# Edresson/VoiceSplit

Measured on AMD Instinct MI355X. Metric: utterances/sec (3 s clips, B=64/GPU) fwd+bwd, channels-last bf16 activations / tape, bf16 MFMA, fp32 accumulate / statistics / master weights, higher is better.
Workload: dtype bf16 (conv activations and tape stored as bf16; bf16 MFMA operands in the convs, the LSTM / head contractions and the BPTT, f16 operands in the forward recurrence; fp32 accumulate, BatchNorm statistics, gate arithmetic / cell state, loss head, master weights)

## Files before the change

### voicesplit_amd/csrc/lstm.hip

```cpp
#include "vs_internal.h"

namespace {

typedef unsigned u32x4_t __attribute__((ext_vector_type(4)));

__global__ void lstm_pack_whh_kernel(const float* __restrict__ whh_f, const float* __restrict__ whh_b,
                                     float* __restrict__ wp, int H) {
  const int HQ = H / 8;
  const long long total = 2LL * HQ * HQ * 256;
  long long idx = (long long)blockIdx.x * blockDim.x + threadIdx.x;
  if (idx >= total) return;
  const int j = idx & 3;
  const int lane = (idx >> 2) & 63;
  long long rest = idx >> 8;
  const int q = rest % HQ; rest /= HQ;
  const int jg = rest % HQ;
  const int dir = rest / HQ;
  const int i = lane & 31;
  const int row = (i >> 3) * H + jg * 8 + (i & 7);
  const int k = 8 * q + 2 * j + (lane >> 5);
  const float* w = dir ? whh_b : whh_f;
  wp[idx] = w[(size_t)row * H + k];
}

// ... 721 lines not shown
    if (s > 0) {
      if (wave == 0 && !sDead) {
        unsigned spins = 0;
        for (;;) {
          bool ok = true;
          for (int j = lane; j < HQ; j += 64)
            ok = ok && (__hip_atomic_load(gflags + j, __ATOMIC_RELAXED, __HIP_MEMORY_SCOPE_AGENT) >= (unsigned)s);
          if (__all(ok)) break;
          if (++spins > kSpinLimit) {
            if (lane == 0) { sDead = 1; __hip_atomic_store(a.err, 1u, __ATOMIC_RELAXED, __HIP_MEMORY_SCOPE_AGENT); }
            break;
          }
          __builtin_amdgcn_s_sleep(1);
        }
      }
      __syncthreads();
      const unsigned hoff = (unsigned)((group * NC * NP * 64 + lane) * 16);
      f16x8 h[kMaxC][NP];
#pragma unroll
      for (int i = 0; i < kMaxC; ++i) {
        const int c = wave + 4 * i;
#pragma unroll
        for (int p = 0; p < NP; ++p)
          h[i][p] = __builtin_bit_cast(f16x8, c < NC ? __builtin_amdgcn_raw_buffer_load_b128(hrs[s & 1], hoff + (unsigned)(c * NP + p) * 1024u, 0, 16 )
                                                       : u32x4_t{0u, 0u, 0u, 0u});
      }
#pragma unroll
      for (int i = 0; i < kMaxC; ++i) {
        if (wave + 4 * i < NC) {
          if (NP == 2) {
            acc = __builtin_amdgcn_mfma_f32_32x32x16_f16(w[i][NP - 1], h[i][0], acc, 0, 0, 0);
            acc = __builtin_amdgcn_mfma_f32_32x32x16_f16(w[i][0], h[i][NP - 1], acc, 0, 0, 0);
          }
          acc = __builtin_amdgcn_mfma_f32_32x32x16_f16(w[i][0], h[i][0], acc, 0, 0, 0);
        }
      }
      for (int c = wave + 4 * kMaxC; c < NC; c += 4) {
        f16x8 wc[NP], hc[NP];
#pragma unroll
        for (int p = 0; p < NP; ++p) {
          wc[p] = __builtin_bit_cast(f16x8, wq[(size_t)(c * NP + p) * 64]);
          hc[p] = __builtin_bit_cast(f16x8, __builtin_amdgcn_raw_buffer_load_b128(hrs[s & 1], hoff + (unsigned)(c * NP + p) * 1024u, 0, 16));
        }
        if (NP == 2) {
          acc = __builtin_amdgcn_mfma_f32_32x32x16_f16(wc[NP - 1], hc[0], acc, 0, 0, 0);
          acc = __builtin_amdgcn_mfma_f32_32x32x16_f16(wc[0], hc[NP - 1], acc, 0, 0, 0);
        }
        acc = __builtin_amdgcn_mfma_f32_32x32x16_f16(wc[0], hc[0], acc, 0, 0, 0);
      }
    }
    if (wave > 0) {
#pragma unroll
      for (int r = 0; r < 16; ++r) sRed[((wave - 1) * 16 + r) * 64 + lane] = acc[r];
    }
    __syncthreads();
    if (wave == 0) {
#pragma unroll
      for (int w3 = 0; w3 < 3; ++w3)
#pragma unroll
        for (int r = 0; r < 16; ++r) acc[r] += sRed[(w3 * 16 + r) * 64 + lane];
      float hv[4], cnew[4], gact[4][4];
#pragma unroll
      for (int u = 0; u < 4; ++u) {
        const float gi = vs_sigmoid_fast(fmaf(acc[0 + u], inv, xgv[0 + u]));
        const float gf = vs_sigmoid_fast(fmaf(acc[4 + u], inv, xgv[4 + u]));
        const float gg = vs_tanh_fast(fmaf(acc[8 + u], inv, xgv[8 + u]));
        const float go = vs_sigmoid_fast(fmaf(acc[12 + u], inv, xgv[12 + u]));
        const float cn = gf * cprev[u] + gi * gg;
        hv[u] = go * vs_tanh_fast(cn);
        cnew[u] = cn;
        cprev[u] = cn;
        gact[0][u] = gi; gact[1][u] = gf; gact[2][u] = gg; gact[3][u] = go;
      }
      {
        float full[8];
#pragma unroll
        for (int u = 0; u < 4; ++u) {
          const float o = __shfl_xor(hv[u], 32, 64);
          full[u] = half ? o : hv[u];
          full[4 + u] = half ? hv[u] : o;
        }
        u32x4_t v;
        typedef _Float16 h2 __attribute__((ext_vector_type(2)));
#pragma unroll
        for (int j = 0; j < 4; ++j) {
          if (NP == 2) {
            const float x0 = full[2 * j] * kHScale, x1 = full[2 * j + 1] * kHScale;
            const h2 hh = __builtin_bit_cast(h2, __builtin_amdgcn_cvt_pkrtz(x0, x1));
            const unsigned lo = __builtin_bit_cast(unsigned, __builtin_amdgcn_cvt_pkrtz(x0 - (float)hh[0], x1 - (float)hh[1]));
            v[j] = half ? lo : __builtin_bit_cast(unsigned, hh);
          } else {
            const h2 hh = {(_Float16)full[2 * j], (_Float16)full[2 * j + 1]};
            v[j] = __builtin_bit_cast(unsigned, hh);
          }
        }
        const unsigned plane = NP == 2 ? (unsigned)half : 0u;
        const unsigned off = (unsigned)((((group * NC + (jg >> 1)) * NP + plane) * 64 + (jg & 1) * 32 + l31) * 16);
        if (NP == 2 || half == 0)
          __builtin_amdgcn_raw_buffer_store_b128(v, hrs[(s + 1) & 1], off, 0, 16 );
      }
      asm volatile("s_waitcnt vmcnt(0)" ::: "memory");
      if (lane == 0) __hip_atomic_store(gflags + jg, (unsigned)(s + 1), __ATOMIC_RELAXED, __HIP_MEMORY_SCOPE_AGENT);
      if (b < a.B) {
        float4* o = reinterpret_cast<float4*>(a.out + ((size_t)b * a.T + t) * (2 * a.H) + (size_t)dir * a.H + jg * 8 + 4 * half);
        *o = make_float4(hv[0], hv[1], hv[2], hv[3]);
        if (a.c_save) {
          float4* cs = reinterpret_cast<float4*>(a.c_save + ((size_t)b * a.T + t) * (2 * a.H) + (size_t)dir * a.H + jg * 8 + 4 * half);
          *cs = make_float4(cnew[0], cnew[1], cnew[2], cnew[3]);
        }
        if (a.gates_save) {
          float* grow = a.gates_save + ((size_t)b * a.T + t) * (8 * a.H) + (size_t)dir * 4 * a.H + jg * 8 + 4 * half;
#pragma unroll
          for (int gq = 0; gq < 4; ++gq)
            *reinterpret_cast<float4*>(grow + gq * a.H) = make_float4(gact[gq][0], gact[gq][1], gact[gq][2], gact[gq][3]);
        }
      }
    }
  }
}

constexpr unsigned kSentinel = 0x7FFF7FFFu;

template <int NP, bool RAGGED>
__global__ __launch_bounds__(256)
void lstm16_tagged_kernel(Lstm16Args a, void* hbuf2, void* hbuf3, const int* __restrict__ lengths) {
  __shared__ float sRed[2][3 * 16 * 64];
  __shared__ int sDead;
  const int tid = threadIdx.x;
  const int lane = tid & 63;
  const int wave = __builtin_amdgcn_readfirstlane(tid >> 6);
  const int l31 = lane & 31, half = lane >> 5;
  const int HQ = a.H / 8;
  const int NC = (a.H + 15) / 16;
  const int NBT = a.Bpad / 32;
  const int jg = blockIdx.x % HQ;
  const int bt = a.bt0 + blockIdx.x / HQ;
  const int dir = blockIdx.y;
  const int b = bt * 32 + l31;
  if (tid == 0) sDead = 0;

  const u32x4_t* wq = a.wp + ((size_t)(dir * HQ + jg) * NC * NP) * 64 + lane;
  f16x8 w[kMaxC][NP];
  bool owned[kMaxC];
#pragma unroll
  for (int i = 0; i < kMaxC; ++i) {
    const int c = wave + 4 * i;
    owned[i] = c < NC && 16 * c + 8 * half < a.H;
#pragma unroll
    for (int p = 0; p < NP; ++p)
      w[i][p] = __builtin_bit_cast(f16x8, c < NC ? wq[(size_t)(c * NP + p) * 64] : u32x4_t{0u, 0u, 0u, 0u});
  }
  const float inv = a.hdr[0];
  const size_t group = (size_t)dir * NBT + bt;
  const unsigned hbytes = (unsigned)((size_t)2 * NBT * NC * NP * 1024);
  __amdgpu_buffer_rsrc_t hrs[4] = {__builtin_amdgcn_make_buffer_rsrc(a.hbuf0, 0, hbytes, 0x00020000),
                                   __builtin_amdgcn_make_buffer_rsrc(a.hbuf1, 0, hbytes, 0x00020000),
                                   __builtin_amdgcn_make_buffer_rsrc(hbuf2, 0, hbytes, 0x00020000),
                                   __builtin_amdgcn_make_buffer_rsrc(hbuf3, 0, hbytes, 0x00020000)};
  const unsigned plane = NP == 2 ? (unsigned)half : 0u;
  const unsigned slot_off = (unsigned)((((group * NC + (jg >> 1)) * NP + plane) * 64 + (jg & 1) * 32 + l31) * 16);
  const bool storer = NP == 2 || half == 0;
  float cprev[4] = {0.f, 0.f, 0.f, 0.f};
  int len = a.T;
  if (RAGGED) len = b < a.B ? lengths[b] : 0;
  __syncthreads();

#pragma unroll 1
  for (int s = 0; s < a.T; ++s) {
    const int t = dir ? (a.T - 1 - s) : s;
    const int rb = s & 3, wb = (s + 1) & 3, zb = (s + 3) & 3;
    float xgv[16];
    if (wave == 0) {
      const bool ok = b < a.B;
      const float* xrow = a.xg + ((size_t)(ok ? b : 0) * a.T + t) * (8 * a.H) + (size_t)dir * 4 * a.H + jg * 8 + 4 * half;
#pragma unroll
      for (int r = 0; r < 16; ++r) xgv[r] = ok ? xrow[(r >> 2) * a.H + (r & 3)] : 0.f;
    }
    f32x16 acc;
#pragma unroll
    for (int r = 0; r < 16; ++r) acc[r] = 0.f;
    if (s > 0) {
      const unsigned hoff = (unsigned)((group * NC * NP * 64 + lane) * 16);
      f16x8 h[kMaxC][NP];
      unsigned spins = 0;
      for (;;) {
        bool ok = true;
#pragma unroll
        for (int i = 0; i < kMaxC; ++i) {
          const int c = wave + 4 * i;
#pragma unroll
          for (int p = 0; p < NP; ++p) {
            u32x4_t v = c < NC ? __builtin_amdgcn_raw_buffer_load_b128(hrs[rb], hoff + (unsigned)(c * NP + p) * 1024u, 0, 16 )
                               : u32x4_t{0u, 0u, 0u, 0u};
            if (!owned[i]) v = u32x4_t{0u, 0u, 0u, 0u};
            ok = ok && v[0] != kSentinel && v[1] != kSentinel && v[2] != kSentinel && v[3] != kSentinel;
            h[i][p] = __builtin_bit_cast(f16x8, v);
          }
        }
        if (__all(ok)) break;
        if (++spins > kSpinLimit / 4 || *(volatile int*)&sDead) {
          if (lane == 0) { sDead = 1; __hip_atomic_store(a.err, 1u, __ATOMIC_RELAXED, __HIP_MEMORY_SCOPE_AGENT); }
          break;
        }
        __builtin_amdgcn_s_sleep(1);
      }
#pragma unroll
      for (int i = 0; i < kMaxC; ++i) {
        if (wave + 4 * i < NC) {
          if (NP == 2) {
            acc = __builtin_amdgcn_mfma_f32_32x32x16_f16(w[i][NP - 1], h[i][0], acc, 0, 0, 0);
            acc = __builtin_amdgcn_mfma_f32_32x32x16_f16(w[i][0], h[i][NP - 1], acc, 0, 0, 0);
          }
          acc = __builtin_amdgcn_mfma_f32_32x32x16_f16(w[i][0], h[i][0], acc, 0, 0, 0);
        }
      }
    }
    if (wave > 0) {
#pragma unroll
      for (int r = 0; r < 16; ++r) sRed[s & 1][((wave - 1) * 16 + r) * 64 + lane] = acc[r];
    }
    if (wave == 1) asm volatile("s_waitcnt vmcnt(0)" ::: "memory");
    __syncthreads();
    if (wave == 1 && s > 0 && storer)
      __builtin_amdgcn_raw_buffer_store_b128(u32x4_t{kSentinel, kSentinel, kSentinel, kSentinel}, hrs[zb], slot_off, 0, 16);
    if (wave == 0) {
#pragma unroll
      for (int w3 = 0; w3 < 3; ++w3)
#pragma unroll
        for (int r = 0; r < 16; ++r) acc[r] += sRed[s & 1][(w3 * 16 + r) * 64 + lane];
      float hv[4], cnew[4], gact[4][4];
#pragma unroll
      for (int u = 0; u < 4; ++u) {
        const float gi = vs_sigmoid_fast(fmaf(acc[0 + u], inv, xgv[0 + u]));
        const float gf = vs_sigmoid_fast(fmaf(acc[4 + u], inv, xgv[4 + u]));
        const float gg = vs_tanh_fast(fmaf(acc[8 + u], inv, xgv[8 + u]));
        const float go = vs_sigmoid_fast(fmaf(acc[12 + u], inv, xgv[12 + u]));
        float cn = gf * cprev[u] + gi * gg;
        hv[u] = go * vs_tanh_fast(cn);
        if (RAGGED) {
          cn = t < len ? cn : 0.f;
          hv[u] = t < len ? hv[u] : 0.f;
        }
        cnew[u] = cn;
        cprev[u] = cn;
        gact[0][u] = gi; gact[1][u] = gf; gact[2][u] = gg; gact[3][u] = go;
      }
      {
        float full[8];
#pragma unroll
        for (int u = 0; u < 4; ++u) {
          const float o = __shfl_xor(hv[u], 32, 64);
          full[u] = half ? o : hv[u];
          full[4 + u] = half ? hv[u] : o;
        }
        u32x4_t v;
        typedef _Float16 h2 __attribute__((ext_vector_type(2)));
#pragma unroll
        for (int j = 0; j < 4; ++j) {
          if (NP == 2) {
            const float x0 = full[2 * j] * kHScale, x1 = full[2 * j + 1] * kHScale;
            const h2 hh = __builtin_bit_cast(h2, __builtin_amdgcn_cvt_pkrtz(x0, x1));
            const unsigned lo = __builtin_bit_cast(unsigned, __builtin_amdgcn_cvt_pkrtz(x0 - (float)hh[0], x1 - (float)hh[1]));
            v[j] = half ? lo : __builtin_bit_cast(unsigned, hh);
          } else {
            const h2 hh = {(_Float16)full[2 * j], (_Float16)full[2 * j + 1]};
            v[j] = __builtin_bit_cast(unsigned, hh);
          }
          v[j] = v[j] == kSentinel ? 0x7FFF7E00u : v[j];
        }
        if (storer) __builtin_amdgcn_raw_buffer_store_b128(v, hrs[wb], slot_off, 0, 16 );
      }
      if (b < a.B) {
        float4* o = reinterpret_cast<float4*>(a.out + ((size_t)b * a.T + t) * (2 * a.H) + (size_t)dir * a.H + jg * 8 + 4 * half);
        *o = make_float4(hv[0], hv[1], hv[2], hv[3]);
        if (a.c_save) {
          float4* cs = reinterpret_cast<float4*>(a.c_save + ((size_t)b * a.T + t) * (2 * a.H) + (size_t)dir * a.H + jg * 8 + 4 * half);
          *cs = make_float4(cnew[0], cnew[1], cnew[2], cnew[3]);
        }
        if (a.gates_save) {
          float* grow = a.gates_save + ((size_t)b * a.T + t) * (8 * a.H) + (size_t)dir * 4 * a.H + jg * 8 + 4 * half;
#pragma unroll
          for (int gq = 0; gq < 4; ++gq)
            *reinterpret_cast<float4*>(grow + gq * a.H) = make_float4(gact[gq][0], gact[gq][1], gact[gq][2], gact[gq][3]);
        }
      }
    }
  }
}

struct Lstm16BwdArgs {
  const u32x4_t* wpt;
  void* gbuf0;
  void* gbuf1;
  unsigned* flags;
  unsigned* err;
  float* gates;
  const float* c_all;
  const float* dout;
  int B, T, H, Bpad, bt0;
};

constexpr int kBwdRes16 = 13;

__global__ __launch_bounds__(512)
void lstm16_bwd_persistent_kernel(Lstm16BwdArgs a) {
  __shared__ float sRed[8 * 16 * 64];
  __shared__ int sDead;
  const int tid = threadIdx.x;
  const int lane = tid & 63;
  const int wave = __builtin_amdgcn_readfirstlane(tid >> 6);
  const int half = lane >> 5;
  const int NCt = a.H / 4;
  const int NUT = (a.H + 31) / 32;
  const int NBT = a.Bpad / 32;
  const int ut = blockIdx.x % NUT;
  const int bt = a.bt0 + blockIdx.x / NUT;
  const int dir = blockIdx.y;
  if (tid == 0) sDead = 0;

  const int b31 = tid & 31, ug = (tid >> 5) & 7;
  const int b = bt * 32 + b31;
  const int u0 = ut * 32 + 4 * ug;
  const bool units_ok = tid < 256 && u0 < a.H;
  const bool item = units_ok && b < a.B;

  const u32x4_t* wq = a.wpt + ((size_t)(dir * NUT + ut) * NCt) * 64 + lane;
  bf16x8 w[kBwdRes16];
#pragma unroll
  for (int i = 0; i < kBwdRes16; ++i) {
    const int c = wave + 8 * i;
    w[i] = __builtin_bit_cast(bf16x8, c < NCt ? wq[(size_t)c * 64] : u32x4_t{0u, 0u, 0u, 0u});
  }
  const size_t group = (size_t)dir * NBT + bt;
  const unsigned gbytes = (unsigned)((size_t)2 * NBT * NCt * 1024);
  __amdgpu_buffer_rsrc_t grs[2] = {__builtin_amdgcn_make_buffer_rsrc(a.gbuf0, 0, gbytes, 0x00020000),
                                   __builtin_amdgcn_make_buffer_rsrc(a.gbuf1, 0, gbytes, 0x00020000)};
  const int nflag = NUT * 4;
  unsigned* const gflags = a.flags + group * nflag;
  float dcc[4] = {0.f, 0.f, 0.f, 0.f};
  __syncthreads();

#pragma unroll 1
  for (int s = 0; s < a.T; ++s) {
    const int t = dir ? s : (a.T - 1 - s);
    const int tp = dir ? t + 1 : t - 1;
    float4 gi4, gf4, gg4, go4, c4, cp4, dh4;
    gi4 = gf4 = gg4 = go4 = c4 = cp4 = dh4 = make_float4(0.f, 0.f, 0.f, 0.f);
    float* grow = a.gates + ((size_t)(item ? b : 0) * a.T + t) * (8 * a.H) + (size_t)dir * 4 * a.H + (item ? u0 : 0);
    if (item) {
      gi4 = *reinterpret_cast<const float4*>(grow);
      gf4 = *reinterpret_cast<const float4*>(grow + a.H);
      gg4 = *reinterpret_cast<const float4*>(grow + 2 * a.H);
      go4 = *reinterpret_cast<const float4*>(grow + 3 * a.H);
      const size_t so = ((size_t)b * a.T + t) * (2 * a.H) + (size_t)dir * a.H + u0;
      c4 = *reinterpret_cast<const float4*>(a.c_all + so);
      dh4 = *reinterpret_cast<const float4*>(a.dout + so);
      if (tp >= 0 && tp < a.T)
        cp4 = *reinterpret_cast<const float4*>(a.c_all + ((size_t)b * a.T + tp) * (2 * a.H) + (size_t)dir * a.H + u0);
    }
    f32x16 acc;
#pragma unroll
    for (int r = 0; r < 16; ++r) acc[r] = 0.f;
    if (s > 0) {
      if (wave == 0 && !sDead) {
        unsigned spins = 0;
        for (;;) {
          bool ok = true;
          for (int j = lane; j < nflag; j += 64)
            ok = ok && (__hip_atomic_load(gflags + j, __ATOMIC_RELAXED, __HIP_MEMORY_SCOPE_AGENT) >= (unsigned)s);
          if (__all(ok)) break;
          if (++spins > kSpinLimit) {
            if (lane == 0) { sDead = 1; __hip_atomic_store(a.err, 1u, __ATOMIC_RELAXED, __HIP_MEMORY_SCOPE_AGENT); }
            break;
          }
          __builtin_amdgcn_s_sleep(1);
        }
      }
      __syncthreads();
      const unsigned goff = (unsigned)((group * NCt * 64 + lane) * 16);
      bf16x8 g[kBwdRes16];
#pragma unroll
      for (int i = 0; i < kBwdRes16; ++i) {
        const int c = wave + 8 * i;
        g[i] = __builtin_bit_cast(bf16x8, c < NCt ? __builtin_amdgcn_raw_buffer_load_b128(grs[s & 1], goff + (unsigned)c * 1024u, 0, 16 )
                                                  : u32x4_t{0u, 0u, 0u, 0u});
      }
#pragma unroll
      for (int i = 0; i < kBwdRes16; ++i) {
        if (wave + 8 * i < NCt)
          acc = __builtin_amdgcn_mfma_f32_32x32x16_bf16(w[i], g[i], acc, 0, 0, 0);
      }
      for (int c = wave + 8 * kBwdRes16; c < NCt; c += 8) {
        const bf16x8 wc = __builtin_bit_cast(bf16x8, wq[(size_t)c * 64]);
        const bf16x8 gc = __builtin_bit_cast(bf16x8, __builtin_amdgcn_raw_buffer_load_b128(grs[s & 1], goff + (unsigned)c * 1024u, 0, 16));
        acc = __builtin_amdgcn_mfma_f32_32x32x16_bf16(wc, gc, acc, 0, 0, 0);
      }
    }
#pragma unroll
    for (int r = 0; r < 16; ++r) sRed[(wave * 16 + r) * 64 + lane] = acc[r];
    __syncthreads();
    if (tid < 256) {
      float dh[4] = {dh4.x, dh4.y, dh4.z, dh4.w};
#pragma unroll
      for (int w8 = 0; w8 < 8; ++w8)
#pragma unroll
        for (int u = 0; u < 4; ++u) dh[u] += sRed[(w8 * 16 + 4 * wave + u) * 64 + lane];
      const float gi[4] = {gi4.x, gi4.y, gi4.z, gi4.w}, gf[4] = {gf4.x, gf4.y, gf4.z, gf4.w};
      const float gg[4] = {gg4.x, gg4.y, gg4.z, gg4.w}, go[4] = {go4.x, go4.y, go4.z, go4.w};
      const float cc[4] = {c4.x, c4.y, c4.z, c4.w}, cp[4] = {cp4.x, cp4.y, cp4.z, cp4.w};
      float dg4[4][4];
#pragma unroll
      for (int u = 0; u < 4; ++u) {
        const float tc = vs_tanh_fast(cc[u]);
        dg4[3][u] = dh[u] * tc * go[u] * (1.f - go[u]);
        const float dc = fmaf(dh[u] * go[u], 1.f - tc * tc, dcc[u]);
        dg4[0][u] = dc * gg[u] * gi[u] * (1.f - gi[u]);
        dg4[1][u] = dc * cp[u] * gf[u] * (1.f - gf[u]);
        dg4[2][u] = dc * gi[u] * (1.f - gg[u] * gg[u]);
        dcc[u] = dc * gf[u];
      }
      if (!item) {
#pragma unroll
        for (int gate = 0; gate < 4; ++gate)
#pragma unroll
          for (int u = 0; u < 4; ++u) dg4[gate][u] = 0.f;
#pragma unroll
        for (int u = 0; u < 4; ++u) dcc[u] = 0.f;
      }
      if (units_ok) {
#pragma unroll
        for (int gate = 0; gate < 4; ++gate) {
          bf16x8 v;
#pragma unroll
          for (int u = 0; u < 4; ++u) {
            const float o = __shfl_xor(dg4[gate][u], 32, 64);
            v[u] = (__bf16)(half ? o : dg4[gate][u]);
            v[4 + u] = (__bf16)(half ? dg4[gate][u] : o);
          }
          const int r0 = gate * a.H + ut * 32 + 8 * wave;
          const unsigned off = (unsigned)(((group * NCt + (r0 >> 4)) * 64 + ((r0 >> 3) & 1) * 32 + b31) * 16);
          if (half == 0)
            __builtin_amdgcn_raw_buffer_store_b128(__builtin_bit_cast(u32x4_t, v), grs[(s + 1) & 1], off, 0, 16 );
        }
      }
      asm volatile("s_waitcnt vmcnt(0)" ::: "memory");
      if (lane == 0) __hip_atomic_store(gflags + ut * 4 + wave, (unsigned)(s + 1), __ATOMIC_RELAXED, __HIP_MEMORY_SCOPE_AGENT);
      if (item) {
        *reinterpret_cast<float4*>(grow) = make_float4(dg4[0][0], dg4[0][1], dg4[0][2], dg4[0][3]);
        *reinterpret_cast<float4*>(grow + a.H) = make_float4(dg4[1][0], dg4[1][1], dg4[1][2], dg4[1][3]);
        *reinterpret_cast<float4*>(grow + 2 * a.H) = make_float4(dg4[2][0], dg4[2][1], dg4[2][2], dg4[2][3]);
        *reinterpret_cast<float4*>(grow + 3 * a.H) = make_float4(dg4[3][0], dg4[3][1], dg4[3][2], dg4[3][3]);
      }
    }
  }
}

}

static size_t lstm_packed_fp32_floats(int H) { return (size_t)2 * (H / 8) * (H / 8) * 256; }
static size_t lstm_packed_f16_floats(int H) { return (size_t)2 * (H / 8) * ((H + 15) / 16) * 2 * 256; }
extern "C" size_t vs_lstm_packed_floats(int H) { return lstm_packed_fp32_floats(H) + lstm_packed_f16_floats(H) + 64; }
static size_t lstm_state_region(int B, int H) { return (size_t)2 * ((H + 15) / 16 * 16) * (((size_t)B + 31) / 32 * 32); }
extern "C" size_t vs_lstm_state_floats(int B, int H) { return 4 * lstm_state_region(B, H) + 64; }

int vs_lstm_pack_impl(const float* whh_f, const float* whh_b, float* wp, int H, hipStream_t stream, int math) {
  VS_REQUIRE(H > 0 && H % 8 == 0, "lstm: hidden size %d must be a multiple of 8", H);
  const long long total = (long long)lstm_packed_fp32_floats(H);
  hipLaunchKernelGGL(lstm_pack_whh_kernel, dim3((unsigned)((total + 255) / 256)), dim3(256), 0, stream, whh_f, whh_b, wp, H);
  VS_LAUNCH_CHECK();
  if (math == VS_MATH_CODE_FP32) return 0;
  u32x4_t* w16 = reinterpret_cast<u32x4_t*>(wp + lstm_packed_fp32_floats(H));
  float* hdr = wp + lstm_packed_fp32_floats(H) + lstm_packed_f16_floats(H);
  const long long slots = 2LL * (H / 8) * ((H + 15) / 16) * 64;
  if (math == VS_MATH_CODE_BF16) {
    hipLaunchKernelGGL((lstm_pack16_kernel<1>), dim3((unsigned)((slots + 255) / 256)), dim3(256), 0, stream, whh_f, whh_b, w16, hdr, H);
  } else {
    unsigned* amax = reinterpret_cast<unsigned*>(hdr + 8);
    VS_CHECK_HIP(hipMemsetAsync(amax, 0, sizeof(unsigned), stream));
    if (int rc = vs_absmax_accum_impl(whh_f, (long long)4 * H * H, amax, stream)) return rc;
    if (int rc = vs_absmax_accum_impl(whh_b, (long long)4 * H * H, amax, stream)) return rc;
    if (int rc = vs_scale_from_absmax_impl(amax, 1, hdr + 1, stream)) return rc;
    hipLaunchKernelGGL((lstm_pack16_kernel<2>), dim3((unsigned)((slots + 255) / 256)), dim3(256), 0, stream, whh_f, whh_b, w16, hdr, H);
  }
  VS_LAUNCH_CHECK();
  return 0;
}

static int g_lstm_kernel = 0;
extern "C" int vs_set_lstm_kernel(int mode) {
  VS_REQUIRE(mode >= 0 && mode <= 4, "vs_set_lstm_kernel: mode %d", mode);
  g_lstm_kernel = mode;
  return 0;
}

namespace {
__global__ void lstm_poison_kernel(const unsigned* __restrict__ err, float* __restrict__ out, int n) {
  if (*err == 0u) return;
  const int i = blockIdx.x * blockDim.x + threadIdx.x;
  if (i < n) out[i] = __uint_as_float(0x7fc00000u);
}

template <class Args>
hipError_t launch_resident(const void* kernel, dim3 grid, dim3 block, Args& a, hipStream_t stream) {
  void* params[] = {&a};
  return hipLaunchCooperativeKernel(kernel, grid, block, params, 0, stream);
}
}

int vs_bilstm_recurrent_impl(const float* xg, const float* wp, float* state, float* out, float* gates_save, float* c_save,
                             int B, int T, int H, hipStream_t stream, int math, const int* lengths) {
  VS_REQUIRE(B > 0 && T > 0 && H > 0 && H % 8 == 0, "lstm: bad shape B=%d T=%d H=%d (H must be a multiple of 8)", B, T, H);
  const int Bpad = (B + 31) / 32 * 32;
  const size_t per = lstm_state_region(B, H);
  if (g_lstm_kernel == 3) math = VS_MATH_CODE_FP32;
  VS_CHECK_HIP(hipMemsetAsync(state, 0, vs_lstm_state_floats(B, H) * sizeof(float), stream));
  float* hbuf[2] = {state, state + per};
  const int HQ = H / 8, NBT = Bpad / 32;
  int dev = 0, cus = 0;
  VS_CHECK_HIP(hipGetDevice(&dev));
  VS_CHECK_HIP(hipDeviceGetAttribute(&cus, hipDeviceAttributeMultiprocessorCount, dev));
  const int bt_per_launch = cus / (2 * HQ);
  const bool persistent = g_lstm_kernel != 1 && bt_per_launch >= 1;
  VS_REQUIRE(g_lstm_kernel != 2 || persistent, "lstm: persistent recurrence needs 2*H/8 = %d workgroups <= %d CUs", 2 * HQ, cus);
  const bool tagged = persistent && math != VS_MATH_CODE_FP32 && g_lstm_kernel != 4 && (H + 15) / 16 <= 4 * kMaxC;
  VS_REQUIRE(!lengths || (tagged && !gates_save && !c_save),
             "lstm: per-item lengths need the tagged persistent recurrence in eval mode (dims.math F16X3 or BF16, H <= %d, 2*H/8 = %d workgroups "
             "<= %d CUs, vs_set_lstm_kernel 0 or 2); VS_MATH_FP32, the flag kernel and the per-step kernels do not take them", 64 * kMaxC, 2 * HQ, cus);
  if (tagged) VS_CHECK_HIP(hipMemsetD32Async(reinterpret_cast<hipDeviceptr_t>(state + per), (int)kSentinel, 3 * per, stream));
  if (persistent) {
    unsigned* flags = reinterpret_cast<unsigned*>(state + 2 * per);
    unsigned* err = reinterpret_cast<unsigned*>(state + 4 * per);
    bool launched = true;
    for (int bt0 = 0; bt0 < NBT; bt0 += bt_per_launch) {
      const int nbt = NBT - bt0 < bt_per_launch ? NBT - bt0 : bt_per_launch;
      hipError_t e;
      if (math == VS_MATH_CODE_FP32) {
        LstmPersistArgs a{xg, wp, hbuf[0], hbuf[1], flags, err, out, gates_save, c_save, B, T, H, Bpad, bt0};
        e = launch_resident(reinterpret_cast<const void*>(&lstm_persistent_kernel), dim3(HQ * nbt, 2), dim3(256), a, stream);
      } else {
        const float* w16 = wp + lstm_packed_fp32_floats(H);
        Lstm16Args a{xg, reinterpret_cast<const u32x4_t*>(w16), w16 + lstm_packed_f16_floats(H), hbuf[0], hbuf[1], flags, err, out,
                     gates_save, c_save, B, T, H, Bpad, bt0};
        if (tagged) {
          void* hb2 = state + 2 * per;
          void* hb3 = state + 3 * per;
          void* params[] = {&a, &hb2, &hb3, &lengths};
          const void* kernel = math == VS_MATH_CODE_BF16
              ? (lengths ? reinterpret_cast<const void*>(&lstm16_tagged_kernel<1, true>) : reinterpret_cast<const void*>(&lstm16_tagged_kernel<1, false>))
              : (lengths ? reinterpret_cast<const void*>(&lstm16_tagged_kernel<2, true>) : reinterpret_cast<const void*>(&lstm16_tagged_kernel<2, false>));
          e = hipLaunchCooperativeKernel(kernel, dim3(HQ * nbt, 2), dim3(256), params, 0, stream);
        } else
        e = math == VS_MATH_CODE_BF16
                ? launch_resident(reinterpret_cast<const void*>(&lstm16_persistent_kernel<1>), dim3(HQ * nbt, 2), dim3(256), a, stream)
                : launch_resident(reinterpret_cast<const void*>(&lstm16_persistent_kernel<2>), dim3(HQ * nbt, 2), dim3(256), a, stream);
      }
      if (e != hipSuccess) {
        (void)hipGetLastError();
        VS_REQUIRE(bt0 == 0 && g_lstm_kernel != 2, "lstm: persistent recurrence could not be launched resident: %s", hipGetErrorString(e));
        VS_REQUIRE(!lengths, "lstm: per-item lengths: the persistent recurrence could not be launched resident (%s) and the per-step kernels do not take them",
                   hipGetErrorString(e));
        launched = false;
        break;
      }
    }
    if (launched) {
      hipLaunchKernelGGL(lstm_poison_kernel, dim3(1), dim3(64), 0, stream, err, out, 64 < B * T * 2 * H ? 64 : B * T * 2 * H);
      VS_LAUNCH_CHECK();
      return 0;
    }
  }
  if (tagged) VS_CHECK_HIP(hipMemsetAsync(state, 0, vs_lstm_state_floats(B, H) * sizeof(float), stream));
  float* c = state + 2 * per;
  dim3 grid(HQ * NBT, 2), block(256);
  for (int s = 0; s < T; ++s) {
    LstmStepArgs a{xg, wp, hbuf[s & 1], hbuf[(s + 1) & 1], c, out, gates_save, c_save, B, T, H, Bpad, s};
    hipLaunchKernelGGL(lstm_step_kernel, grid, block, 0, stream, a);
  }
  VS_LAUNCH_CHECK();
  return 0;
}

static size_t lstm_packed_t_fp32_floats(int H) { return (size_t)2 * ((H + 31) / 32) * (H / 2) * 256; }
static size_t lstm_packed_t_bf16_floats(int H) { return (size_t)2 * ((H + 31) / 32) * (H / 4) * 256; }
extern "C" size_t vs_lstm_packed_t_floats(int H) { return lstm_packed_t_fp32_floats(H) + lstm_packed_t_bf16_floats(H) + 64; }
extern "C" size_t vs_lstm_bwd_state_floats(int B, int H) {
  const size_t Bpad = ((size_t)B + 31) / 32 * 32;
  return 2 * (2 * (Bpad / 32) * (size_t)(H / 2) * 256) + 2 * Bpad * H + 64;
}

int vs_lstm_pack_t_impl(const float* whh_f, const float* whh_b, float* wp, int H, hipStream_t stream, int math) {
  VS_REQUIRE(H > 0 && H % 8 == 0, "lstm: hidden size %d must be a multiple of 8", H);
  const long long total = (long long)lstm_packed_t_fp32_floats(H);
  hipLaunchKernelGGL(lstm_pack_whh_t_kernel, dim3((unsigned)((total + 255) / 256)), dim3(256), 0, stream, whh_f, whh_b, wp, H);
  VS_LAUNCH_CHECK();
  if (math != VS_MATH_CODE_BF16) return 0;
  const long long slots = 2LL * ((H + 31) / 32) * (H / 4) * 64;
  hipLaunchKernelGGL(lstm_pack16_t_kernel, dim3((unsigned)((slots + 255) / 256)), dim3(256), 0, stream, whh_f, whh_b,
                     reinterpret_cast<u32x4_t*>(wp + lstm_packed_t_fp32_floats(H)), H);
  VS_LAUNCH_CHECK();
  return 0;
}

int vs_bilstm_bwd_recurrent_impl(const float* wpt, float* state, float* gates, const float* c_all, const float* dout,
                                 int B, int T, int H, hipStream_t stream, int math) {
  VS_REQUIRE(B > 0 && T > 0 && H > 0 && H % 8 == 0, "lstm_bwd: bad shape B=%d T=%d H=%d (H must be a multiple of 8)", B, T, H);
  if (g_lstm_kernel == 3) math = VS_MATH_CODE_FP32;
  const int Bpad = (B + 31) / 32 * 32;
  const size_t frag = (size_t)2 * (Bpad / 32) * (H / 2) * 256;
  VS_CHECK_HIP(hipMemsetAsync(state, 0, vs_lstm_bwd_state_floats(B, H) * sizeof(float), stream));
  float* gbuf[2] = {state, state + frag};
  const int NUT = (H + 31) / 32, NBT = Bpad / 32;
  int dev = 0, cus = 0;
  VS_CHECK_HIP(hipGetDevice(&dev));
  VS_CHECK_HIP(hipDeviceGetAttribute(&cus, hipDeviceAttributeMultiprocessorCount, dev));
  const int bt_per_launch = cus / (2 * NUT);
  const bool persistent = g_lstm_kernel != 1 && bt_per_launch >= 1;
  VS_REQUIRE(g_lstm_kernel != 2 || persistent, "lstm_bwd: persistent recurrence needs %d workgroups <= %d CUs", 2 * NUT, cus);
  if (persistent) {
    unsigned* flags = reinterpret_cast<unsigned*>(state + 2 * frag);
    unsigned* err = reinterpret_cast<unsigned*>(state + 2 * frag + (size_t)2 * Bpad * H);
    bool launched = true;
    for (int bt0 = 0; bt0 < NBT; bt0 += bt_per_launch) {
      const int nbt = NBT - bt0 < bt_per_launch ? NBT - bt0 : bt_per_launch;
      hipError_t e;
      if (math == VS_MATH_CODE_BF16) {
        Lstm16BwdArgs a{reinterpret_cast<const u32x4_t*>(wpt + lstm_packed_t_fp32_floats(H)), gbuf[0], gbuf[1], flags, err, gates, c_all, dout,
                        B, T, H, Bpad, bt0};
        e = launch_resident(reinterpret_cast<const void*>(&lstm16_bwd_persistent_kernel), dim3(NUT * nbt, 2), dim3(512), a, stream);
      } else {
        LstmBwdPersistArgs a{wpt, gbuf[0], gbuf[1], flags, err, gates, c_all, dout, B, T, H, Bpad, bt0};
        e = launch_resident(reinterpret_cast<const void*>(&lstm_bwd_persistent_kernel), dim3(NUT * nbt, 2), dim3(512), a, stream);
      }
      if (e != hipSuccess) {
        (void)hipGetLastError();
        VS_REQUIRE(bt0 == 0 && g_lstm_kernel != 2, "lstm_bwd: persistent recurrence could not be launched resident: %s", hipGetErrorString(e));
        launched = false;
        break;
      }
    }
    if (launched) {
      hipLaunchKernelGGL(lstm_poison_kernel, dim3(1), dim3(64), 0, stream, err, gates, 64 < B * T * 8 * H ? 64 : B * T * 8 * H);
      VS_LAUNCH_CHECK();
      return 0;
    }
  }
  if (persistent) VS_CHECK_HIP(hipMemsetAsync(state, 0, vs_lstm_bwd_state_floats(B, H) * sizeof(float), stream));
  float* dc = state + 2 * frag;
  dim3 grid(NUT * NBT, 2), block(512);
  for (int s = 0; s < T; ++s) {
    LstmBwdArgs a{wpt, gbuf[s & 1], gbuf[(s + 1) & 1], gates, c_all, dout, dc, B, T, H, Bpad, s};
    hipLaunchKernelGGL(lstm_bwd_step_kernel, grid, block, 0, stream, a);
  }
  VS_LAUNCH_CHECK();
  return 0;
}
```

Before: 1421.

## Remap BPTT thread-to-unit layout for coalesced tape loads in bf16 LSTM backward

Adds a templated variant of the persistent bf16 BPTT kernel that maps threads so consecutive lanes cover consecutive hidden units of one batch row. Per-step gate, cell and dout tape reads then coalesce into contiguous lines rather than strided per-batch accesses. To fit the new mapping it XOR-swizzles the shared-memory reduction buffer to avoid bank conflicts and repacks the bf16 gate-gradient fragments with a lane shuffle before the buffer stores. The new layout becomes the default, and the old layout stays reachable through mode 6. The extra shuffle and index arithmetic sit on the serial recurrence critical path.

```diff
diff --git a/voicesplit_amd/csrc/lstm.hip b/voicesplit_amd/csrc/lstm.hip
--- a/voicesplit_amd/csrc/lstm.hip
+++ b/voicesplit_amd/csrc/lstm.hip
@@ -1047,6 +1047,27 @@
 
 constexpr int kBwdRes16 = 13;
 
+struct BpttTape {
+  float4 gi, gf, gg, go, c, cp, dh;
+};
+
+__device__ __forceinline__ void bptt_tape_load(BpttTape& r, const Lstm16BwdArgs& a, int dir, int s, int brow, int ucol) {
+  const int t = dir ? s : (a.T - 1 - s);
+  const int tp = dir ? t + 1 : t - 1;
+  const bool has_prev = tp >= 0 && tp < a.T;
+  const float* grow = a.gates + ((size_t)brow * a.T + t) * (8 * a.H) + (size_t)dir * 4 * a.H + ucol;
+  const size_t so = ((size_t)brow * a.T + t) * (2 * a.H) + (size_t)dir * a.H + ucol;
+  r.gi = *reinterpret_cast<const float4*>(grow);
+  r.gf = *reinterpret_cast<const float4*>(grow + a.H);
+  r.gg = *reinterpret_cast<const float4*>(grow + 2 * a.H);
+  r.go = *reinterpret_cast<const float4*>(grow + 3 * a.H);
+  r.c = *reinterpret_cast<const float4*>(a.c_all + so);
+  r.dh = *reinterpret_cast<const float4*>(a.dout + so);
+  const float4 cp = *reinterpret_cast<const float4*>(a.c_all + ((size_t)brow * a.T + (has_prev ? tp : t)) * (2 * a.H) + (size_t)dir * a.H + ucol);
+  r.cp = has_prev ? cp : make_float4(0.f, 0.f, 0.f, 0.f);
+}
+
+template <bool kLine>
 __global__ __launch_bounds__(512)
 void lstm16_bwd_persistent_kernel(Lstm16BwdArgs a) {
   __shared__ float sRed[8 * 16 * 64];
@@ -1063,11 +1084,14 @@
   const int dir = blockIdx.y;
   if (tid == 0) sDead = 0;
 
-  const int b31 = tid & 31, ug = (tid >> 5) & 7;
+  const int b31 = kLine ? (tid >> 3) & 31 : tid & 31, ug = kLine ? tid & 7 : (tid >> 5) & 7;
   const int b = bt * 32 + b31;
   const int u0 = ut * 32 + 4 * ug;
   const bool units_ok = tid < 256 && u0 < a.H;
   const bool item = units_ok && b < a.B;
+  const bool gate_wave = wave < 4;
+  const int rrow = 4 * (ug >> 1);
+  const int rcol = (32 * (ug & 1) + b31) ^ (8 * (ug >> 1) + 4 * (ug & 1));
 
   const u32x4_t* wq = a.wpt + ((size_t)(dir * NUT + ut) * NCt) * 64 + lane;
   bf16x8 w[kBwdRes16];
@@ -1083,25 +1107,29 @@
   const int nflag = NUT * 4;
   unsigned* const gflags = a.flags + group * nflag;
   float dcc[4] = {0.f, 0.f, 0.f, 0.f};
+  const float4 zero4 = make_float4(0.f, 0.f, 0.f, 0.f);
   __syncthreads();
 
 #pragma unroll 1
   for (int s = 0; s < a.T; ++s) {
     const int t = dir ? s : (a.T - 1 - s);
     const int tp = dir ? t + 1 : t - 1;
-    float4 gi4, gf4, gg4, go4, c4, cp4, dh4;
-    gi4 = gf4 = gg4 = go4 = c4 = cp4 = dh4 = make_float4(0.f, 0.f, 0.f, 0.f);
+    BpttTape tape{zero4, zero4, zero4, zero4, zero4, zero4, zero4};
     float* grow = a.gates + ((size_t)(item ? b : 0) * a.T + t) * (8 * a.H) + (size_t)dir * 4 * a.H + (item ? u0 : 0);
-    if (item) {
-      gi4 = *reinterpret_cast<const float4*>(grow);
-      gf4 = *reinterpret_cast<const float4*>(grow + a.H);
-      gg4 = *reinterpret_cast<const float4*>(grow + 2 * a.H);
-      go4 = *reinterpret_cast<const float4*>(grow + 3 * a.H);
-      const size_t so = ((size_t)b * a.T + t) * (2 * a.H) + (size_t)dir * a.H + u0;
-      c4 = *reinterpret_cast<const float4*>(a.c_all + so);
-      dh4 = *reinterpret_cast<const float4*>(a.dout + so);
-      if (tp >= 0 && tp < a.T)
-        cp4 = *reinterpret_cast<const float4*>(a.c_all + ((size_t)b * a.T + tp) * (2 * a.H) + (size_t)dir * a.H + u0);
+    if (!kLine) {
+      if (item) {
+        tape.gi = *reinterpret_cast<const float4*>(grow);
+        tape.gf = *reinterpret_cast<const float4*>(grow + a.H);
+        tape.gg = *reinterpret_cast<const float4*>(grow + 2 * a.H);
+        tape.go = *reinterpret_cast<const float4*>(grow + 3 * a.H);
+        const size_t so = ((size_t)b * a.T + t) * (2 * a.H) + (size_t)dir * a.H + u0;
+        tape.c = *reinterpret_cast<const float4*>(a.c_all + so);
+        tape.dh = *reinterpret_cast<const float4*>(a.dout + so);
+        if (tp >= 0 && tp < a.T)
+          tape.cp = *reinterpret_cast<const float4*>(a.c_all + ((size_t)b * a.T + tp) * (2 * a.H) + (size_t)dir * a.H + u0);
+      }
+    } else if (gate_wave) {
+      bptt_tape_load(tape, a, dir, s, item ? b : 0, item ? u0 : 0);
     }
     f32x16 acc;
 #pragma unroll
@@ -1142,17 +1170,17 @@
       }
     }
 #pragma unroll
-    for (int r = 0; r < 16; ++r) sRed[(wave * 16 + r) * 64 + lane] = acc[r];
+    for (int r = 0; r < 16; ++r) sRed[(wave * 16 + r) * 64 + (kLine ? lane ^ (8 * (r >> 2) + 4 * half) : lane)] = acc[r];
     __syncthreads();
     if (tid < 256) {
-      float dh[4] = {dh4.x, dh4.y, dh4.z, dh4.w};
+      float dh[4] = {tape.dh.x, tape.dh.y, tape.dh.z, tape.dh.w};
 #pragma unroll
       for (int w8 = 0; w8 < 8; ++w8)
 #pragma unroll
-        for (int u = 0; u < 4; ++u) dh[u] += sRed[(w8 * 16 + 4 * wave + u) * 64 + lane];
-      const float gi[4] = {gi4.x, gi4.y, gi4.z, gi4.w}, gf[4] = {gf4.x, gf4.y, gf4.z, gf4.w};
-      const float gg[4] = {gg4.x, gg4.y, gg4.z, gg4.w}, go[4] = {go4.x, go4.y, go4.z, go4.w};
-      const float cc[4] = {c4.x, c4.y, c4.z, c4.w}, cp[4] = {cp4.x, cp4.y, cp4.z, cp4.w};
+        for (int u = 0; u < 4; ++u) dh[u] += kLine ? sRed[(w8 * 16 + rrow + u) * 64 + rcol] : sRed[(w8 * 16 + 4 * wave + u) * 64 + lane];
+      const float gi[4] = {tape.gi.x, tape.gi.y, tape.gi.z, tape.gi.w}, gf[4] = {tape.gf.x, tape.gf.y, tape.gf.z, tape.gf.w};
+      const float gg[4] = {tape.gg.x, tape.gg.y, tape.gg.z, tape.gg.w}, go[4] = {tape.go.x, tape.go.y, tape.go.z, tape.go.w};
+      const float cc[4] = {tape.c.x, tape.c.y, tape.c.z, tape.c.w}, cp[4] = {tape.cp.x, tape.cp.y, tape.cp.z, tape.cp.w};
       float dg4[4][4];
 #pragma unroll
       for (int u = 0; u < 4; ++u) {
@@ -1172,7 +1200,33 @@
 #pragma unroll
         for (int u = 0; u < 4; ++u) dcc[u] = 0.f;
       }
-      if (units_ok) {
+      if (kLine) {
+        unsigned own[8];
+#pragma unroll
+        for (int gate = 0; gate < 4; ++gate) {
+          bf16x8 v;
+#pragma unroll
+          for (int u = 0; u < 4; ++u) { v[u] = (__bf16)dg4[gate][u]; v[4 + u] = (__bf16)0.f; }
+          const u32x4_t p = __builtin_bit_cast(u32x4_t, v);
+          own[2 * gate] = p[0];
+          own[2 * gate + 1] = p[1];
+        }
+        const bool odd = ug & 1;
+        unsigned keep[4], got[4];
+#pragma unroll
+        for (int i = 0; i < 4; ++i) {
+          keep[i] = odd ? own[4 + i] : own[i];
+          got[i] = (unsigned)__shfl_xor((int)(odd ? own[i] : own[4 + i]), 1, 64);
+        }
+#pragma unroll
+        for (int j = 0; j < 2; ++j) {
+          const unsigned k0 = keep[2 * j], k1 = keep[2 * j + 1], g0 = got[2 * j], g1 = got[2 * j + 1];
+          const u32x4_t v = {odd ? g0 : k0, odd ? g1 : k1, odd ? k0 : g0, odd ? k1 : g1};
+          const int r0 = ((odd ? 2 : 0) + j) * a.H + ut * 32 + 8 * (ug >> 1);
+          const unsigned off = (unsigned)(((group * NCt + (r0 >> 4)) * 64 + ((r0 >> 3) & 1) * 32 + b31) * 16);
+          if (units_ok) __builtin_amdgcn_raw_buffer_store_b128(v, grs[(s + 1) & 1], off, 0, 16 );
+        }
+      } else if (units_ok) {
 #pragma unroll
         for (int gate = 0; gate < 4; ++gate) {
           bf16x8 v;
@@ -1233,7 +1287,7 @@
 
 static int g_lstm_kernel = 0;
 extern "C" int vs_set_lstm_kernel(int mode) {
-  VS_REQUIRE(mode >= 0 && mode <= 4, "vs_set_lstm_kernel: mode %d", mode);
+  VS_REQUIRE((mode >= 0 && mode <= 4) || mode == 6, "vs_set_lstm_kernel: mode %d", mode);
   g_lstm_kernel = mode;
   return 0;
 }
@@ -1371,7 +1425,9 @@
       if (math == VS_MATH_CODE_BF16) {
         Lstm16BwdArgs a{reinterpret_cast<const u32x4_t*>(wpt + lstm_packed_t_fp32_floats(H)), gbuf[0], gbuf[1], flags, err, gates, c_all, dout,
                         B, T, H, Bpad, bt0};
-        e = launch_resident(reinterpret_cast<const void*>(&lstm16_bwd_persistent_kernel), dim3(NUT * nbt, 2), dim3(512), a, stream);
+        const void* kernel = g_lstm_kernel == 6 ? reinterpret_cast<const void*>(&lstm16_bwd_persistent_kernel<false>)
+                                                : reinterpret_cast<const void*>(&lstm16_bwd_persistent_kernel<true>);
+        e = launch_resident(kernel, dim3(NUT * nbt, 2), dim3(512), a, stream);
       } else {
         LstmBwdPersistArgs a{wpt, gbuf[0], gbuf[1], flags, err, gates, c_all, dout, B, T, H, Bpad, bt0};
         e = launch_resident(reinterpret_cast<const void*>(&lstm_bwd_persistent_kernel), dim3(NUT * nbt, 2), dim3(512), a, stream);
```

Result: no change. 1431 (median of 6 runs) (+0.7%).
